# thu-wangz17/HermNet

Measured on AMD Instinct MI355X. Metric: atom-steps/sec (energy+forces) on 10k-atom 3-element cell; HBM GB/s vs roofline, higher is better.
Workload: dtype f32; 1 GPU; configs[1]: 10000-atom 3-element fcc alloy (Al/Ni/Cu), HVNet rc=5.0 hidden=128 num_rbf=128 layers=5, E=431340 directed edges, energy+forces per step; config=c2, atoms_total=10000, atoms_owned_rank0=10000, halo_atoms_rank0=0, edges_rank0=431340, tuned_gemm_table=False, gemm_tuning_in_warmup=False, parallelism=1 GPU

## Files before the change

### hermnet_amd/csrc/message_bwd_cl.hip

```cpp
#include <hip/hip_runtime.h>
#include <stdint.h>
#include <type_traits>
#include "../../include/hermnet_hip.h"
#include "hermnet_math.h"
#include "message_bwd_cl.h"

namespace {

typedef float hn_f2 __attribute__((ext_vector_type(2)));
typedef unsigned hn_u2 __attribute__((ext_vector_type(2)));
typedef __attribute__((address_space(4))) const float hn_cfloat;
typedef __attribute__((address_space(4))) const int hn_cint;

constexpr int kRec = HN_EDGE_TABLE_FLOATS;

#ifndef HN_NT_TABLE
#define HN_NT_TABLE 1
#endif
__device__ __forceinline__ float fwd_envelope_val(float u, int kind, int p) {
#pragma clang fp contract(off)
  if (kind != 0 || !(u < 1.0f)) return hn_envelope(u, kind, p).val;
  const float up = hn_powi(u, p - 1) * u;
  const float w = 1.0f - u;
  const float fp = (float)p;
// ... 332 lines not shown
    }
    for (int base = e_begin; base < e_end; base += 64) {
      const int cnt = min(64, e_end - base);
      const unsigned my_off = lane < cnt ? (unsigned)a.csc_tgt[base + lane] * (unsigned)(H * 4) : 0u;
      const int my_pos = lane < cnt ? a.csc_pos[base + lane] : 0;

      auto load_edge = [&](int k) {
        EdgeIn in;
        const unsigned so = (unsigned)__builtin_amdgcn_readlane((int)my_off, k);
        in.gx1 = buf_load(rs_gx1, c4, so);
        in.g0 = buf_load(rs_gvec1, c4, 3u * so);
        in.g1 = buf_load(rs_gvec1, c4, 3u * so + h4);
        in.g2 = buf_load(rs_gvec1, c4, 3u * so + 2 * h4);
        return in;
      };

      EdgeIn in0 = load_edge(0), in1 = in0;
      float px[2], py[2], pz[2];
      float ux[2], uy[2], uz[2];
      auto edge_body = [&](auto J, int k) {
        constexpr int j = decltype(J)::value;
        while (base + k >= row_end) {
          row_epilogue(row);
          ++row;
          row_end = row_end2;
          row_end2 = rowptr_c[min(row + 2, a.Nsrc)];
          row_request(row);
        }
        const int kn = j == 3 ? min(k + 1, 63) : k + 1;
        if (j & 1) in0 = load_edge(kn); else in1 = load_edge(kn);
        const EdgeIn& cur = (j & 1) ? in1 : in0;
        float (&tl)[5] = (j & 1) ? tl1 : tl0;
        hn_f2 Ss = {0.f, 0.f}, Sa = {0.f, 0.f}, Sb = {0.f, 0.f};
        auto taps4 = [&](int m0, const hn_f4 (&w)[4]) {
#pragma unroll
          for (int q = 0; q < 4; ++q) {
            const hn_f2 g = {rec[2 * (m0 + q)], rec[2 * (m0 + q) + 1]};
            Ss = __builtin_elementwise_fma(g, hn_f2{w[q].x, w[q].x}, Ss);
            if (HAS_VEC) Sa = __builtin_elementwise_fma(g, hn_f2{w[q].y, w[q].y}, Sa);
            Sb = __builtin_elementwise_fma(g, hn_f2{w[q].z, w[q].z}, Sb);
          }
        };
        lds_wait_all(wA, wB, wC);
#if HN_KO_BWD == 1
        Ss = hn_f2{rec[0] * wA[0].x, rec[1]}; Sa = hn_f2{rec[2] * wB[0].y, rec[3]}; Sb = hn_f2{rec[4] * wC[0].z, rec[5]};
#else
        taps4(0, wA);
        taps4(4, wB);
        taps4(8, wC);
#endif
        unsigned waddr_next;
        float own = 1.0f;
        if constexpr (WIN) {
          const int prow_next = __float_as_int(tl[0]);
          waddr_next = (unsigned)win_row(prow_next) * (HN_CB * 16) + tile_lane;
          own = own_cur ? 1.0f : 0.0f;
          own_mask = j == 0 ? own_cur : (own_mask | (own_cur << j));
          own_cur = win_owns(prow_next);
        } else {
          waddr_next = (unsigned)__float_as_int(tl[0]) * (HN_CB * 16) + tile_lane;
        }
        __builtin_amdgcn_sched_barrier(0);
        asm volatile("" : "+v"(Ss), "+v"(Sa), "+v"(Sb));
        rp += kRec;
        if (j & 1) load_record(tl0); else load_record(tl1);
        issue_weights(waddr_next);
        __builtin_amdgcn_sched_barrier(0);
        if (fresh) row_scale();
#if HN_KO_BWD == 2
        {
          gs += Ss.x + Ss.y + cur.gx1; ga += Sa.x + Sa.y + cur.g0; gb += Sb.x + Sb.y + cur.g1 + cur.g2;
          px[j & 1] = gs; py[j & 1] = ga; pz[j & 1] = gb;
          return;
        }
#endif
        const float rx = tl[1], ry = tl[2], rz = tl[3], invd = tl[4];
        const float gx1 = WIN ? cur.gx1 * own : cur.gx1, g0 = WIN ? cur.g0 * own : cur.g0;
        const float g1 = WIN ? cur.g1 * own : cur.g1, g2 = WIN ? cur.g2 * own : cur.g2;
        const float rs = Ss.x + bs;
        if (NEED_GXH) gs = fmaf(gx1, rs, gs);
        float pdv = gx1 * xs * Ss.y;
        if (HAS_VEC) {
          const float ra_ = Sa.x + ba;
          const float A = fmaf(g0, vj0, fmaf(g1, vj1, g2 * vj2));
          ga = fmaf(A, ra_, ga);
          const float w = xas * ra_;
          gv0 = fmaf(g0, w, gv0); gv1 = fmaf(g1, w, gv1); gv2 = fmaf(g2, w, gv2);
          pdv = fmaf(A * xa, Sa.y, pdv);
        }
        const float rb_ = Sb.x + bb;
        const float B = fmaf(rx, g0, fmaf(ry, g1, rz * g2));
        if (NEED_GXH) gb = fmaf(B, rb_, gb);
        pdv = fmaf(B * xb, Sb.y, pdv);
        const float qi = xb * rb_ * invd;
        const float tpar = fmaf(-B, qi, pdv);
        px[j & 1] = fmaf(tpar, rx, g0 * qi); py[j & 1] = fmaf(tpar, ry, g1 * qi); pz[j & 1] = fmaf(tpar, rz, g2 * qi);
      };
      auto fold = [&](int h) {
        ux[h] = pair_fold(px[0], px[1]); uy[h] = pair_fold(py[0], py[1]); uz[h] = pair_fold(pz[0], pz[1]);
      };
      auto group_store = [&](int k4) {
        const float sx = quad_total(ux[0], ux[1]), sy = quad_total(uy[0], uy[1]), sz = quad_total(uz[0], uz[1]);
        const int je = (row16 == 0) ? 0 : (row16 == 1 ? 2 : (row16 == 2 ? 1 : 3));
        const int p0 = __builtin_amdgcn_readlane(my_pos, k4), p1 = __builtin_amdgcn_readlane(my_pos, min(k4 + 1, cnt - 1));
        const int p2 = __builtin_amdgcn_readlane(my_pos, min(k4 + 2, cnt - 1)), p3 = __builtin_amdgcn_readlane(my_pos, min(k4 + 3, cnt - 1));
        const int pw = (row16 == 0) ? p0 : (row16 == 1 ? p2 : (row16 == 2 ? p1 : p3));
        if constexpr (WIN) {
          if ((lane & 15) == 0 && k4 + je < cnt && ((own_mask >> je) & 1u)) gedge[pw] = make_float4(sx, sy, sz, 0.f);
        } else {
#if HN_NT_MSG
          if ((lane & 15) == 0 && k4 + je < cnt)
            __builtin_nontemporal_store(hn_f4{sx, sy, sz, 0.f}, reinterpret_cast<hn_f4*>(&gedge[pw]));
#else
          if ((lane & 15) == 0 && k4 + je < cnt) gedge[pw] = make_float4(sx, sy, sz, 0.f);
// ... 202 lines not shown
```

### hermnet_amd/csrc/node_kernels.hip

```cpp
#include <hip/hip_runtime.h>
#include "../../include/hermnet_hip.h"

namespace {

constexpr float kInvSqrt2 = 0.70710678118654752f;
constexpr float kSiluScale = 1.0f / 0.6f;

__device__ __forceinline__ float4 ld4(const float* p) { return *reinterpret_cast<const float4*>(p); }
__device__ __forceinline__ void st4(float* p, float4 v) { *reinterpret_cast<float4*>(p) = v; }
__device__ __forceinline__ float sigmoidf_(float x) { return 1.0f / (1.0f + __expf(-x)); }


__device__ __forceinline__ float4 add4(float4 a, float4 b) { return make_float4(a.x + b.x, a.y + b.y, a.z + b.z, a.w + b.w); }

__device__ __forceinline__ float4 bias4(const float* bias, int rows_per_bias, long row, int cols, int col) {
  if (bias == nullptr) return make_float4(0.f, 0.f, 0.f, 0.f);
  const long grp = rows_per_bias > 0 ? row / rows_per_bias : 0;
  return ld4(bias + grp * cols + col);
}

__global__ __launch_bounds__(256) void ssilu_fwd_kernel(const float* __restrict__ h, const float* __restrict__ bias,
                                                        int rows_per_bias, float* __restrict__ a, long n4, int cols) {
  const long i = (long)blockIdx.x * blockDim.x + threadIdx.x;
  if (i >= n4) return;
// ... 457 lines not shown
                                                        const int* __restrict__ ranges, int num_ranges) {
  const int q4 = H;
  const long i = (long)blockIdx.x * blockDim.x + threadIdx.x;
  const long rows = MODE == 0 ? rows_out : (MODE == 1 ? (long)Te * P * B : (long)Te * B);
  if (i >= rows * q4) return;
  const long r = i / q4;
  if (MODE == 2 && num_ranges > 0) {
    bool in = false;
    for (int k = 0; k < num_ranges; ++k) in |= r >= ranges[2 * k] && r < ranges[2 * k + 1];
    if (!in) return;
  }
  const int c = (int)(i % q4) * 4;
  const float sc = c < H ? sx : sv;
  auto at = [&](const float* x, const float* v, long row) {
    return c < H ? ld4(x + row * H + c) : ld4(v + row * 3 * H + (c - H));
  };
  float* dst = c < H ? xout + r * H + c : vout + r * 3 * H + (c - H);
  if (MODE != 1) {
    float4 acc = make_float4(0.f, 0.f, 0.f, 0.f);
    if (r < (long)Te * B) {
      const long ce = r / B, ii = r % B;
      for (int k = 0; k < P; ++k) acc = add4(acc, at(xin, vin, (ce * P + k) * B + ii));
      acc = make_float4(acc.x * sc, acc.y * sc, acc.z * sc, acc.w * sc);
    }
    if (MODE == 2) acc = add4(acc, ld4(dst));
    st4(dst, acc);
  } else {
    const long ce = r / ((long)P * B), ii = r % B;
    const float4 g = at(xin, vin, ce * B + ii);
    st4(dst, make_float4(g.x * sc, g.y * sc, g.z * sc, g.w * sc));
  }
}

inline dim3 grid_for(long n, int block) { return dim3((unsigned)((n + block - 1) / block)); }
#define HN_LAUNCH_END return hipGetLastError() == hipSuccess ? HN_OK : HN_ERR_LAUNCH

}

extern "C" int hermnet_ssilu_fwd(const float* h, const float* bias, int rows_per_bias, float* a, long rows, int cols,
                                 void* stream) {
  if (rows < 0 || cols <= 0 || (cols & 3)) return HN_ERR_BAD_ARG;
  if (rows == 0) return HN_OK;
  if (!h || !a) return HN_ERR_BAD_ARG;
  const long n4 = rows * (cols / 4);
  hipLaunchKernelGGL(ssilu_fwd_kernel, grid_for(n4, 256), dim3(256), 0, (hipStream_t)stream, h, bias, rows_per_bias,
                     a, n4, cols);
  HN_LAUNCH_END;
}

extern "C" int hermnet_ssilu_bwd(const float* g, const float* h, const float* bias, int rows_per_bias, float* gh,
                                 int N, int T, int C, long g_stride_n, long g_stride_t, void* stream) {
  if (N < 0 || T <= 0 || C <= 0 || (C & 3) || (g_stride_n & 3) || (g_stride_t & 3)) return HN_ERR_BAD_ARG;
  if (N == 0) return HN_OK;
  if (!g || !h || !gh) return HN_ERR_BAD_ARG;
  hipLaunchKernelGGL(ssilu_bwd_kernel, grid_for((long)N * T * (C / 4), 256), dim3(256), 0, (hipStream_t)stream,
                     g, h, bias, rows_per_bias, gh, N, T, C, g_stride_n, g_stride_t);
  HN_LAUNCH_END;
}

extern "C" int hermnet_update_mid(const float* vp, const float* x1, float* vdot, float* xin, int rows, int hidden,
                                  void* stream) {
  if (rows < 0 || hidden <= 0 || (hidden & 3)) return HN_ERR_BAD_ARG;
  if (rows == 0) return HN_OK;
  if (!vp || !x1 || !vdot || !xin) return HN_ERR_BAD_ARG;
  hipLaunchKernelGGL(update_mid_kernel, grid_for((long)rows * (hidden / 4), 256), dim3(256), 0, (hipStream_t)stream,
                     vp, x1, vdot, xin, rows, hidden);
// ... 104 lines not shown
  };
  if (cols == 64) return go(energy_head_fused_kernel<true, 1>);
  if (cols == 128) return go(energy_head_fused_kernel<true, 2>);
  return go(energy_head_fused_kernel<true, 4>);
}

extern "C" int hermnet_energy_head_fused_bwd(const float* ge, const float* h, const float* w0, const float* w2,
                                             const float* row_mask, float* gx, int rows, int hidden, int cols,
                                             void* stream) {
  if (rows < 0 || (hidden != 64 && hidden != 128 && hidden != 256) || cols <= 0 || (cols & 3) ||
      (size_t)hidden * cols * 4 > 65536)
    return HN_ERR_BAD_ARG;
  if (rows == 0) return HN_OK;
  if (!ge || !h || !w0 || !w2 || !gx) return HN_ERR_BAD_ARG;
  const size_t lds = ((size_t)hidden * cols + 32 * (cols + 1)) * sizeof(float);
  const dim3 grid((unsigned)((rows + 31) / 32));
  hipStream_t s = (hipStream_t)stream;
  auto go = [&](auto kern) -> int {
    static bool done = false;
    if (!done) {
      if (hipFuncSetAttribute(reinterpret_cast<const void*>(kern), hipFuncAttributeMaxDynamicSharedMemorySize, 98304) != hipSuccess)
        return HN_ERR_LDS;
      done = true;
    }
    hipLaunchKernelGGL(kern, grid, dim3(256), lds, s, h, w0, (const float*)nullptr, w2, (const float*)nullptr, ge, row_mask,
                       gx, (float*)nullptr, rows, cols);
    HN_LAUNCH_END;
  };
  if (hidden == 64) return go(energy_head_fused_kernel<false, 1>);
  if (hidden == 128) return go(energy_head_fused_kernel<false, 2>);
  return go(energy_head_fused_kernel<false, 4>);
}

extern "C" int hermnet_pair_mean(int mode, const float* x_in, const float* vec_in, float* x_out, float* vec_out,
                                 int num_elem, int pairs, int block, int rows_out, int hidden, float scale_x,
                                 float scale_vec, const int* row_ranges, int num_ranges, void* stream) {
  if (num_elem < 0 || pairs <= 0 || block < 0 || hidden <= 0 || (hidden & 3) || rows_out < (long)num_elem * block ||
      mode < 0 || mode > 2 || num_ranges < 0 || (num_ranges > 0 && (!row_ranges || mode != 2)))
    return HN_ERR_BAD_ARG;
  const long rows = mode == 0 ? (long)rows_out : (mode == 1 ? (long)num_elem * pairs * block : (long)num_elem * block);
  if (rows == 0) return HN_OK;
  if (!x_in || !vec_in || !x_out || !vec_out) return HN_ERR_BAD_ARG;
  const dim3 grid = grid_for(rows * hidden, 256);
  hipStream_t s = (hipStream_t)stream;
  switch (mode) {
    case 0: hipLaunchKernelGGL(pair_mean_kernel<0>, grid, dim3(256), 0, s, x_in, vec_in, x_out, vec_out, num_elem, pairs, block, rows_out, hidden, scale_x, scale_vec, (const int*)nullptr, 0); break;
    case 1: hipLaunchKernelGGL(pair_mean_kernel<1>, grid, dim3(256), 0, s, x_in, vec_in, x_out, vec_out, num_elem, pairs, block, rows_out, hidden, scale_x, scale_vec, (const int*)nullptr, 0); break;
    default: hipLaunchKernelGGL(pair_mean_kernel<2>, grid, dim3(256), 0, s, x_in, vec_in, x_out, vec_out, num_elem, pairs, block, rows_out, hidden, scale_x, scale_vec, row_ranges, num_ranges); break;
  }
  HN_LAUNCH_END;
}

extern "C" int hermnet_halo_rows(int mode, float* x, float* vec, const long* idx, int n, int hidden, float* buf,
                                 void* stream) {
  if (n < 0 || hidden <= 0 || (hidden & 3) || mode < 0 || mode > 2) return HN_ERR_BAD_ARG;
  if (n == 0) return HN_OK;
  if (!x || !vec || !idx || !buf) return HN_ERR_BAD_ARG;
  const dim3 grid = grid_for((long)n * hidden, 256);
  hipStream_t s = (hipStream_t)stream;
  switch (mode) {
    case 0: hipLaunchKernelGGL(halo_rows_kernel<0>, grid, dim3(256), 0, s, x, vec, idx, n, hidden, buf); break;
    case 1: hipLaunchKernelGGL(halo_rows_kernel<1>, grid, dim3(256), 0, s, x, vec, idx, n, hidden, buf); break;
    case 2: hipLaunchKernelGGL(halo_rows_kernel<2>, grid, dim3(256), 0, s, x, vec, idx, n, hidden, buf); break;
    default: return HN_ERR_BAD_ARG;
  }
  HN_LAUNCH_END;
// ... 39 lines not shown
```

### hermnet_amd/hermnet.py

```python
from typing import Dict, List, Union

import torch
from torch import nn

from . import nodeops, switches
from .elements import atomic_numbers
from .ops import EdgeGeometry, TrueEdgeGradient, edge_radial_tables
from .relations import AtomSet, RelationalGraph
from .sharding import HaloExchange, HaloExchangeFeatures, HaloGradReturn, SumAcrossRanks
from .layer import (EdgeFanout, EdgeGradSink, EnergyHead, FusedRelationalLayer, GemmRelationalLayer, HeadWeights, LayerWeights,
                    Route, StepState)
from .rmnet import PaiNNModule, RadialBasis, ScaledSiLU, relational_layer
from .trainops import EdgeDiff, EdgeUnit, embedding_rows, tall_linear


class HeteroVertexConv(nn.Module):

    def __init__(self, mods: Dict[str, nn.Module]):
        super().__init__()
        self.mods = nn.ModuleDict(mods)
        self._weights = None

    def forward(self, data):
        step = data.get("_hn_step")
        if step is None:
            raise RuntimeError("HeteroVertexConv.forward needs a Data prepared by HVNet.forward")
        g, li = step.graph, step.layer
        halo, step.halo = step.halo, None
        ready = step.weights
        w = ready[li] if (ready is not None and ready[li].mods[0] is next(iter(self.mods.values()))) else None
        if w is None and step.edge_embed is None and switches.fused_layer:
            if self._weights is None:
                self._weights = LayerWeights(self.mods.values())
            w = self._weights.refresh()
        if halo is not None and _exchange_first(halo, w, g, data.x):
            data.x, data.vec = HaloExchangeFeatures.apply(data.x, data.vec, halo.plan)
            halo = None
        if step.edge_embed is not None:
            data.x, data.vec = relational_layer(self.mods.values(), data.x, data.vec, step.edge, g, None,
                                                edge_embed=step.edge_embed)
            return data
        if not switches.fused_layer:
            data.x, data.vec = relational_layer(self.mods.values(), data.x, data.vec, step.edge, g, step.rbf)
            return data
        edge = step.edge if step.edge_handles is None else step.edge_handles[li]
        node, step.chain_node = step.chain_node, None
        if not (w.chain and switches.node_chain):
            if halo is not None:
                raise RuntimeError("the in-layer halo exchange belongs to the chain path")
            data.x, data.vec = GemmRelationalLayer.apply(data.x, data.vec, edge, g, step.rbf, w, step)
            return data
        route = _chain_route(data, step, node, halo)
        data.x, data.vec = FusedRelationalLayer.apply(data.x, data.vec, edge, g, step.rbf, w, step, route)
        step.chain_node = None if g.num_src else data.x.grad_fn
        return data


def _exchange_first(halo, w, g, x):
    return not (w is not None and w.chain and switches.node_chain
                and halo.fwd_early is not None and g.N * 3 * x.size(1) * 4 < 2 ** 32
                and sum(halo.plan.recv_counts) + sum(halo.plan.send_counts) > 0
                and switches.halo_overlap() != "0")


def _chain_route(data, step, node, halo):
    g, li, ready = step.graph, step.layer, step.weights
    straight = (node is not None and data.vec is not None and data.x.grad_fn is node and data.vec.grad_fn is node
                and not g.num_src and not torch.is_anomaly_enabled()
                and not getattr(data.x, "_backward_hooks", None) and not getattr(data.vec, "_backward_hooks", None))
    if halo is not None:
        return Route("proj" if straight and switches.halo_overlap() not in ("0", "1") else "rows", halo)
    pre = step.pre_next.pop(li, None)
    if pre is not None and not (pre[0].data_ptr() == data.x.data_ptr() and pre[0].shape == data.x.shape):
        pre = None
    w_next = ready[li + 1] if (ready is not None and li + 1 < len(ready) and step.whole) else None
    last = step.last and not g.num_src and w_next is None
    return Route(defer=straight and step.whole, pre=None if pre is None else pre[1], w_next=w_next, last=last)


class GraphEnergies(torch.autograd.Function):

    @staticmethod
    def forward(ctx, e_rows, graph, batch):
        ctx.graph, ctx.batch, ctx.rows = graph, batch, e_rows.size(0)
        pa = e_rows.index_select(0, graph.row_of_node).index_select(0, graph.graph_perm)
        return torch.segment_reduce(pa, "sum", lengths=graph.graph_lengths, unsafe=True)

    @staticmethod
    def backward(ctx, ge):
        return _GraphSpread.apply(ge, ctx.graph, ctx.batch, ctx.rows), None, None


class _GraphSpread(torch.autograd.Function):
    @staticmethod
    def forward(ctx, ge, graph, batch, rows):
        ctx.graph, ctx.batch = graph, batch
        def make():
            idx = torch.zeros(rows, dtype=torch.long, device=ge.device).scatter_(0, graph.row_of_node, batch)
            real = torch.zeros(rows, dtype=ge.dtype, device=ge.device).scatter_(
                0, graph.row_of_node, torch.ones(graph.row_of_node.numel(), dtype=ge.dtype, device=ge.device))
            return idx, real
        idx, real = graph.derived("row_graph", make, key=rows)
        return ge.index_select(0, idx) * real

    @staticmethod
    def backward(ctx, c_rows):
        return GraphEnergies.apply(c_rows.contiguous(), ctx.graph, ctx.batch), None, None, None


MAX_PADDED_WIDTH = 1024
# ... 3 lines not shown

    def __init__(self, elems: Union[str, List[str]], rc: float = 5.,
                 intensive: bool = False, num_layers: int = 5,
                 hidden_channels: int = 512, num_rbf: int = 128,
                 rbf={"name": "gaussian"},
                 envelope={"name": "polynomial", "exponent": 5}):
        super().__init__()
        if isinstance(elems, str):
            elems = [elems]
        self.elems = list(elems)
        if (hidden_channels + 63) // 64 * 64 > MAX_PADDED_WIDTH:
            raise ValueError("hermnet_amd: hidden_channels = %d pads to %d channels; the LayerNorm kernels hold a row of at "
                             "most %d (csrc/node_kernels.hip: kLnMaxPerLane), so the widest model has hidden_channels = %d"
                             % (hidden_channels, (hidden_channels + 63) // 64 * 64, MAX_PADDED_WIDTH, MAX_PADDED_WIDTH))
        self.rc = rc
        self.num_layers = num_layers
        self.hidden_channels = hidden_channels
        self.intensive = intensive

        self.embed = nn.Embedding(len(atomic_numbers), hidden_channels)
        self.radial_basis = RadialBasis(num_radial=num_rbf, cutoff=rc, rbf=rbf, envelope=envelope)
        self.hermconvs = nn.ModuleList()
        for _ in range(num_layers):
            self.hermconvs.append(HeteroVertexConv(
                mods={ntype: PaiNNModule(hidden_channels=hidden_channels, num_rbf=num_rbf) for ntype in self.elems}))
        self.out_energy = nn.Sequential(
            nn.Linear(hidden_channels, hidden_channels // 2),
            ScaledSiLU(),
            nn.Linear(hidden_channels // 2, 1),
        )

    def invalidate_caches(self):
        self.__dict__["_cache_epoch"] = self.__dict__.get("_cache_epoch", 0) + 1
        for w in [getattr(conv, "_weights", None) for conv in self.hermconvs] + [self.__dict__.get("_head")]:
            if w is not None:
                w.key = None
        g = self.__dict__.get("_guard")
        if g is not None:
            g.armed_for, g._event = None, None
        return self

    def load_state_dict(self, *args, **kwargs):
        out = super().load_state_dict(*args, **kwargs)
        self.invalidate_caches()
        return out

    def _apply(self, fn, *args, **kwargs):
        out = super()._apply(fn, *args, **kwargs)
        if "hermconvs" in self._modules:
            self.invalidate_caches()
        return out

    def train(self, mode=True):
        if "hermconvs" in self._modules and mode != self.training:
            self.invalidate_caches()
        return super().train(mode)

    def _refresh_weights(self, dev):
        from .guard import ParamGuard
        guard_on = dev.type == "cuda" and switches.param_guard()
        for _ in range(2):
            ws = []
            for conv in self.hermconvs:
                if conv._weights is None:
                    conv._weights = LayerWeights(conv.mods.values())
                ws.append(conv._weights.refresh())
            hw = None
            if (self.hidden_channels // 2) % 4 == 0:
                if self.__dict__.get("_head") is None:
                    self.__dict__["_head"] = HeadWeights(self.out_energy)
                hw = self._head.refresh()
            if not guard_on or not ws:
                return ws, hw
            g = self.__dict__.get("_guard")
            if g is None:
                g = self.__dict__["_guard"] = ParamGuard(self)
            extra = tuple((p_.data_ptr(), p_._version) for p_ in (self.embed.weight, self.out_energy[0].weight,
                                                                 self.out_energy[0].bias, self.out_energy[2].weight,
                                                                 self.out_energy[2].bias))
            if not g.step(dev, tuple((id(w), w.builds) for w in ws + [hw] if w is not None) + extra, ws[0].b1cat):
                return ws, hw
            self.invalidate_caches()
        return ws, hw

    eval_param_grads = False

    @staticmethod
    def _require_device(pos):
        if not pos.is_cuda:
            raise RuntimeError("hermnet_amd.HVNet runs on MI355X only (data is on %s); there is no CPU fallback"
                               % pos.device)

    def _require_fp32(self, pos):
        wd = self.embed.weight.dtype
        if wd != torch.float32 or pos.dtype != torch.float32:
            raise TypeError("hermnet_amd.HVNet computes in float32: parameters are %s, data.pos is %s "
                            "(call model.float() / pos.float())" % (wd, pos.dtype))

    def _z_list(self):
        return [atomic_numbers[el] for el in self.elems]

    def atom_set(self, atomic_number, batch):
        return AtomSet.of(atomic_number, batch, self._z_list())

    def _build_graph(self, data, zl, shard, atoms):
        rel_active = None if shard is None else shard.rel_active(zl)
        return RelationalGraph.build(data.atomic_number, data.edge_index, zl,
                                     edge_shift=data.get("edge_shift") if data.get("cell") is not None else None,
                                     batch=data.batch, rel_active=rel_active, atoms=atoms)

    @staticmethod
    def _edge_geometry_autograd(pos, cell, graph):
        src = graph.src_id.long()
# ... 65 lines not shown
        if train and pos.is_cuda:
            x = embedding_rows(self.embed.weight, graph.z_rows.long())
        else:
            x = self.embed(graph.z_rows) if train else torch.nn.functional.embedding(graph.z_rows, self.embed.weight.detach())
        H = self.hidden_channels
        Hp = (H + 63) // 64 * 64 if (fused and switches.fused_layer) else H
        if Hp != H:
            x = torch.nn.functional.pad(x, (0, Hp - H))
        weights, head = self._refresh_weights(pos.device) if fused and switches.fused_layer else (None, None)
        if train:
            edge, edge_parts = self._edge_geometry_autograd(pos, data.get("cell"), graph)
        elif props is not None and (props.want_virials or props.want_graph_virial):
            edge = EdgeGeometry.apply(pos, data.get("cell"), graph, props)
        else:
            edge = EdgeGeometry.apply(pos, data.get("cell"), graph)
        if not fused and not train:
            edge = TrueEdgeGradient.apply(edge)
        graph.fwd_taps = None
        if fused and edge.requires_grad and edge.is_cuda:
            graph.edge_table, graph.fwd_taps = edge_radial_tables(graph, rbf, edge.detach())
        if fused:
            edge_embed = None
        elif train and pos.is_cuda and self.radial_basis.rbf_name == "gaussian" and H % 4 == 0 and graph.T > 0:
            parts, Ek = edge_parts, graph.rel_edge_total()
            edge_embed = self.radial_basis.bucketed(edge[:, 3] if parts is None else parts[1], Ek, graph.T,
                                                    graph.rel_edge_bounds_dev())
            if parts is not None:
                edge_embed.set_unit_vectors(edge, parts[0], Ek)
        else:
            edge_embed = self.radial_basis(edge[:, 3])
        data.x, data.vec = x, None
        data._hn_graph, data._hn_edge, data._hn_edge_embed = graph, edge, edge_embed
        step = StepState(graph, edge, rbf, edge_embed, train=train, fused=fused, whole=whole, weights=weights, head=head)
        if fused and edge.requires_grad and switches.fused_layer:
            all_known = graph.num_src == 0 and graph.N == graph.type_rowptr_host[-1]
            step.edge_sink = EdgeGradSink(len(self.hermconvs), Hp // 64, graph.E, pos.device, zero=not all_known)
            step.edge_handles = EdgeFanout.apply(edge, step.edge_sink)
        return step

    def _run_layers(self, data, step):
        graph, edge, L = step.graph, step.edge, len(self.hermconvs)
        for li, conv in enumerate(self.hermconvs):
            step.layer = li
            step.last = bool(li + 1 == L and step.fused and switches.fused_layer and switches.dead_ends
                             and type(conv) is HeteroVertexConv
                             and edge.requires_grad and not conv._forward_hooks
                             and not torch.nn.modules.module._global_forward_hooks)
            data = conv(data)
            if not step.whole and li + 1 < L:
                step.halo = data._hn_shard.halo_overlap(graph, nodeops.chain_tile_rows(data.x.size(1)) or 64)
        step.weights = step.edge_handles = step.halo = step.chain_node = None
        return data

    def _read_out(self, data, step):
        graph, shard, H = step.graph, data.get("_hn_shard"), self.hidden_channels
        x = data.x if data.x.size(1) == H else data.x[:, :H]
        head, step.head = step.head, None
        mask = graph.row_real if shard is None and graph.num_graphs == 1 else None
        if shard is not None and shard.num_graphs == 1 and head is not None:
            mask = shard.owned_rows(graph, x.size(0))
        e_rows = self._row_energies(x, step.train, head, mask)
        props = data.get("_hn_atom_props")
        if props is not None and props.want_energies:
            props.energies = self._atom_energies(e_rows, graph, data.batch)
        return self._graph_energies(e_rows, graph, data.batch, shard, mask is not None)

# ... 124 lines not shown
```

### hermnet_amd/layer.py

```python
import torch

from . import _lib, nodeops, switches
from .ops import _launch, _msg_bwd, _msg_bwd_gedge, _msg_fwd
from .sharding import _all_to_all_rows_start, comm_wait


class LayerWeights(object):

    STATE = ("mods", "key", "builds", "_params", "h_real", "chain")
    DENSE = ("w1cat", "b1cat", "w1cat_t", "w2", "w2t", "b2", "wt", "brbf", "wv", "wvt", "wx0", "wx0t", "bx0", "wx2", "wx2t",
             "bx2", "wv_s", "wvt_s", "wx0_s", "wx0t_s", "bx0_s", "wx2_s", "wx2t_s", "bx2_s")
    FRAG = ("w1f", "w1tf", "w2f", "w2tf", "wvf", "wvtf", "wx0f", "wx0tf", "wx2f", "wx2tf")
    FRAG16 = tuple(n + "16" for n in FRAG)
    __slots__ = STATE + DENSE + FRAG + FRAG16

    def __init__(self, mods):
        for n in self.__slots__:
            setattr(self, n, None)
        self.mods = list(mods)
        self.builds = 0
        self._params = [(sub, name) for m in self.mods for sub in m.modules() for name in sub._parameters]

    @property
    def __dict__(self):
# ... 73 lines not shown
    return tuple(key)


class HeadWeights(object):

    __slots__ = ("lin0", "lin2", "key", "builds", "w0", "b0", "w2v", "b2", "w0t", "w0f16", "w0tf16")

    def __init__(self, out_energy=None):
        for n in self.__slots__:
            setattr(self, n, None)
        if out_energy is not None:
            self.lin0, self.lin2 = out_energy[0], out_energy[2]
        self.builds = 0

    @torch.no_grad()
    def refresh(self):
        key = _version_key([(m, n) for m in (self.lin0, self.lin2) for n in ("weight", "bias")])
        if key != self.key:
            self.build(self.lin0.weight.detach(), self.lin0.bias.detach(), self.lin2.weight.detach(), self.lin2.bias.detach())
            self.key = key
            self.builds += 1
        return self

    def build(self, w0, b0, w2, b2):
        H, C = w0.size(1), w0.size(0)
        self.w0, self.b0, self.w2v, self.b2 = w0.contiguous(), b0, w2.reshape(-1).contiguous(), b2
        if nodeops.head16_supported(H, C):
            self.w0f16, self.w0tf16 = nodeops.weight_fragments16(self.w0), nodeops.weight_fragments16(self.w0.t().contiguous())
        elif nodeops.head_fused_supported(H, C):
            self.w0t = self.w0.t().contiguous()
        return self


def _bwd_sums_deferrable(graph, H):
    return (H == 128 and graph.edge_table is not None and not graph.num_src and graph.res_row is None
            and _lib.get_option("bwd_lanes16") == 0
            and graph.N * 3 * H * 4 < 2 ** 32 and switches.defer_sums())


def _virtual_residual(graph, gx1, gvec1, gx_in, gvec_in, H, ranges=None):
    if not graph.num_src:
        return
    P_, B_, Te = graph.triadic_pairs, graph.block, graph.T // graph.triadic_pairs
    if gx_in.is_cuda and gvec_in is not None:
        nodeops.pair_sum_accumulate(gx1, gvec1, gx_in, gvec_in, Te, P_, B_, 0.5 ** 0.5, 1.0, ranges=ranges)
        return
    sel = slice(0, Te * B_)
    if ranges is not None:
        sel = torch.zeros(Te * B_, dtype=torch.bool)
        for lo, hi in ranges[1]:
            sel[lo:min(hi, Te * B_)] = True
    gx_in[:Te * B_][sel] += (gx1.view(Te, P_, B_, H).sum(1).reshape(Te * B_, H) * (0.5 ** 0.5))[sel]
    if gvec_in is not None:
        gvec_in[:Te * B_][sel] += gvec1.view(Te, P_, B_, 3, H).sum(1).reshape(Te * B_, 3, H)[sel]


class EdgeGradSink(object):

    def __init__(self, layers, nblk, E, device, zero=True):
        self.shape = (layers, nblk, E, 4)
        self.device = device
        self.zero = zero
        self.buf = None

    def slice(self, li):
        if self.buf is None:
            alloc = torch.zeros if self.zero else torch.empty
            self.buf = alloc(self.shape, dtype=torch.float32, device=self.device)
            if not self.zero and switches.debug_poison():
                self.buf.fill_(float("nan"))
        return self.buf[li]


class EdgeFanout(torch.autograd.Function):

    @staticmethod
    def forward(ctx, edge, sink):
        ctx.sink = sink
        L, nblk = sink.shape[0], sink.shape[1]
        return tuple(edge.unsqueeze(0).expand(nblk, *edge.shape) for _ in range(L))

    @staticmethod
    def backward(ctx, *grads):
        sink = ctx.sink
        buf, ctx.sink.buf = sink.buf, None
        if buf is not None and all(g is not None and g.data_ptr() == buf[i].data_ptr() for i, g in enumerate(grads)):
            L, nblk, E, _ = sink.shape
            return buf.view(L * nblk, E, 4).sum(0), None
        live = [g.sum(0) for g in grads if g is not None]
        return (torch.stack(live, 0).sum(0) if live else None), None


class StepState(object):

    __slots__ = ("graph", "edge", "rbf", "edge_embed", "train", "fused", "whole", "weights", "head", "edge_sink",
                 "edge_handles", "layer", "last", "halo", "chain_node", "pending", "pre_next")

    def __init__(self, graph=None, edge=None, rbf=None, edge_embed=None, train=False, fused=False, whole=True, weights=None,
                 head=None):
        self.graph = graph
        self.edge = edge
        self.rbf = rbf
        self.edge_embed = edge_embed
        self.train = train
        self.fused = fused
        self.whole = whole
        self.weights = weights
        self.head = head
        self.edge_sink = None
        self.edge_handles = None
        self.layer = 0
        self.last = False
        self.halo = None
        self.chain_node = None
        self.pending = {}
        self.pre_next = {}


class Route(object):

    def __init__(self, exchange=None, halo=None, defer=False, pre=None, w_next=None, last=False):
        self.exchange, self.halo, self.defer, self.pre, self.w_next = exchange, halo, defer, pre, w_next
        self.boundary = int(switches.boundary_mode)
        self.first = bool(switches.dead_ends)
        self.last = bool(last and switches.dead_ends and exchange is None and w_next is None)


def _local_fwd(x, vec, edge, graph, rbf, w, route):
    pre = route.pre if route.pre is not None else nodeops.node_pre_fwd(x, w, graph.T, src_ranges=graph.src_ranges)
    x1, vec1 = _msg_fwd(graph, rbf, x.size(1), pre[1], vec, x, w, edge, xh_bias=False)
    return pre, x1, vec1


def _halo_rows_fwd(x, vec, edge, graph, rbf, w, route):
    halo, plan, H = route.halo, route.halo.plan, x.size(1)
    send = nodeops.halo_rows(0, x, vec, plan.send_idx)
    recv, work = _all_to_all_rows_start(send, plan.send_counts, plan.recv_counts, plan.group)
    if switches.debug_poison():
        nodeops.halo_rows(2, x, vec, plan.recv_idx, torch.full_like(recv, float("nan")))
    pre = nodeops.node_pre_fwd(x, w, graph.T, src_ranges=graph.src_ranges)
    out = _msg_fwd(graph, rbf, H, pre[1], vec, x, w, edge, xh_bias=False, ranges=halo.fwd_early, zero_unknown=True,
                   range_rows=halo.early_rows)
    comm_wait(work, "fwd", sum(plan.send_counts), sum(plan.recv_counts))
    if plan.recv_idx.numel() > 0:
        nodeops.halo_rows(2, x, vec, plan.recv_idx, recv)
        nodeops.node_pre_fwd(x, w, graph.T, src_ranges=graph.src_ranges, windows=halo.windows, mode=1, out=pre)
    if halo.late_rows > 0:
        _msg_fwd(graph, rbf, H, pre[1], vec, x, w, edge, xh_bias=False, ranges=halo.fwd_late, zero_unknown=False, out=out,
                 range_rows=halo.late_rows)
    return pre, out[0], out[1]


def _halo_proj_fwd(x, vec, edge, graph, rbf, w, route):
    halo, plan, H = route.halo, route.halo.plan, x.size(1)
    pre = nodeops.node_pre_fwd(x, w, graph.T, src_ranges=graph.src_ranges)
    xh = pre[1]
    send = nodeops.halo_proj_rows(0, xh, vec, plan.send_idx)
    recv, work = _all_to_all_rows_start(send, plan.send_counts, plan.recv_counts, plan.group)
    if switches.debug_poison():
        nodeops.halo_proj_rows(2, xh, vec, plan.recv_idx, torch.full_like(recv, float("nan")))
    out = _msg_fwd(graph, rbf, H, xh, vec, x, w, edge, xh_bias=False, ranges=halo.fwd_early, zero_unknown=True,
                   range_rows=halo.early_rows)
# ... 91 lines not shown
    return gx_total, gvec_in


def _halo_proj_bwd(ctx, x, mean, rstd, hb, xh, vec, edge, gx1, gvec1, gedge):
    graph, rbf, w, halo, plan, H = ctx.graph, ctx.rbf, ctx.w, ctx.route.halo, ctx.route.halo.plan, x.size(1)
    gxh = torch.empty_like(xh)
    gv_parts = torch.empty((graph.T,) + tuple(vec.shape), dtype=vec.dtype, device=vec.device)
    bufs = (gxh, gv_parts)
    if halo.bwd_first_rows[1]:
        _msg_bwd(graph, rbf, H, xh, vec, w, edge, gx1, gvec1, gedge, xh_bias=False, ranges=halo.bwd_first_rows, out=bufs,
                 finish=False)
    gsend = nodeops.halo_proj_rows(1, gxh, gv_parts, plan.recv_idx)
    back, work = _all_to_all_rows_start(gsend, plan.recv_counts, plan.send_counts, plan.group)
    if halo.bwd_rest_rows[1]:
        _msg_bwd(graph, rbf, H, xh, vec, w, edge, gx1, gvec1, gedge, xh_bias=False, ranges=halo.bwd_rest_rows, out=bufs,
                 finish=False)
    comm_wait(work, "bwd", sum(plan.recv_counts), sum(plan.send_counts))
    nodeops.halo_proj_accumulate(gxh, gv_parts, plan, back)
    gn_parts = nodeops.node_pre_bwd(gxh, hb, x, mean, rstd, w, src_ranges=graph.src_ranges, parts_only=True)
    return _hand_down(ctx.step, ctx.li, x, vec, gn_parts, gv_parts, mean, rstd, gx1, gvec1, w)


_ROUTES = {None: (_local_fwd, _local_bwd), "rows": (_halo_rows_fwd, _halo_rows_bwd), "proj": (_halo_proj_fwd, _halo_proj_bwd)}


class FusedRelationalLayer(torch.autograd.Function):

    @staticmethod
    def forward(ctx, x, vec, edge, graph, rbf, w, step, route):
        x = x.contiguous()
        vec = None if vec is None else vec.contiguous()
        ctx.exchange = "rows" if (route.exchange == "proj" and not _bwd_sums_deferrable(graph, x.size(1))
                                  and (ctx.needs_input_grad[0] or ctx.needs_input_grad[2])) else route.exchange
        (hb, xh, mean, rstd), x1, vec1 = _ROUTES[ctx.exchange][0](x, vec, edge, graph, rbf, w, route)
        ctx.short = route.last and x.is_cuda and ctx.exchange is None and nodeops.last_update_supported(graph, x.size(1), w)
        if ctx.short:
            x_out, vp, h2b, q23, nrm = nodeops.node_update_fwd_last(x1, vec1, w, graph)
            vec_out = None
        else:
            x_out, vec_out, vp, h2b, q23, nrm = _update_fwd(x1, vec1, graph, w, step, step.layer, route)
        ctx.save_for_backward(x, mean, rstd, hb, xh, vec, edge, vp, h2b, q23, nrm)
        ctx.graph, ctx.rbf, ctx.w, ctx.step, ctx.li, ctx.route = graph, rbf, w, step, step.layer, route
        return x_out, vec_out

    @staticmethod
    def backward(ctx, gxo, gvo):
        x, mean, rstd, hb, xh, vec, edge, vp, h2b, q23, nrm = ctx.saved_tensors
        pend = ctx.step.pending.pop(ctx.li, None)
        if ctx.short:
            if pend is not None:
                raise RuntimeError("hermnet_amd: gradients handed down to the last layer")
            gx1, gvec1 = nodeops.node_update_bwd_last(gxo.contiguous(), vp, h2b, q23, nrm, ctx.w, ctx.graph)
        else:
            gxo, gvo = gxo.contiguous(), gvo.contiguous()
            if pend is not None and (pend.gx.data_ptr() != gxo.data_ptr() or pend.gvec.data_ptr() != gvo.data_ptr()):
                raise RuntimeError("hermnet_amd: the gradients handed down as partial sums (layer %d) did not arrive in the "
                                   "buffers they were registered with; set the environment variable named in "
                                   "hermnet_amd/switches.py: defer_sums to 0" % (ctx.li + 1))
            gx1, gvec1 = nodeops.node_update_bwd(gxo, gvo, vp, h2b, q23, nrm, ctx.w, ctx.graph, pending=pend)
        gedge = _edge_grad_slot(edge, ctx.graph, ctx.step, ctx.li, x.size(1), gx1.device)
        gx, gvec = _ROUTES[ctx.exchange][1](ctx, x, mean, rstd, hb, xh, vec, edge, gx1, gvec1, gedge)
        return (gx, gvec, _edge_grad(edge, gedge)) + (None,) * 5


def _relation_gemms(graph, a, w_s, w_t, out, bias=None, acc=False):
    rp = graph.type_rowptr_host
# ... 107 lines not shown
```

### hermnet_amd/nodeops.py

```python

import ctypes

import torch

from . import _lib
from .ops import _call

P = _lib.ptr


def _new(like, *shape):
    return torch.empty(*shape, dtype=like.dtype, device=like.device)


def layernorm_fwd(x, eps=1e-5, h_real=0):
    rows, H = x.shape
    n, mean, rstd = _new(x, rows, H), _new(x, rows), _new(x, rows)
    _call("layernorm_fwd", "hermnet_layernorm_fwd", P(x), P(n), P(mean), P(rstd), rows, H, h_real, eps)
    return n, mean, rstd


def layernorm_bwd(g, x, mean, rstd, add=None, h_real=0):
    rows, H = x.shape
    gx = _new(x, rows, H)
# ... 179 lines not shown
def update_tile_rows(graph, H):
    return graph.derived("upd_tile", lambda: int(_lib.load().hermnet_node_update_tile_rows(
        _rowptr_host(graph), graph.N, graph.T, H)), key=H)


def update_stream(graph, H, w):
    if update_tile_rows(graph, H) == 16 and w.wvf16 is not None:
        return _stream16(w)
    return 0, (w.wvf, w.wx0f, w.wx2f), (w.wx2tf, w.wx0tf, w.wvtf)


def _stream16(w):
    return 16, (w.wvf16, w.wx0f16, w.wx2f16), (w.wx2tf16, w.wx0tf16, w.wvtf16)


def _rowptr_host(graph):
    return graph.derived("rowptr_c", lambda: (ctypes.c_int * len(graph.type_rowptr_host))(*graph.type_rowptr_host))


def _pre_outputs(x, T, zero_stats=False):
    Ns, H = x.shape
    alloc = torch.zeros if zero_stats else torch.empty
    hb, xh = _new(x, T, Ns, H), _new(x, T, Ns, 3 * H)
    return hb, xh, alloc(Ns, dtype=x.dtype, device=x.device), alloc(Ns, dtype=x.dtype, device=x.device)


def node_pre_fwd(x, w, T, src_ranges=None, windows=None, mode=0, out=None):
    Ns, H = x.shape
    hb, xh, mean, rstd = out if out is not None else _pre_outputs(x, T, zero_stats=src_ranges is not None)
    nwin = 0 if windows is None else int(windows.size(0))
    _call("node_pre_fwd", "hermnet_node_pre_fwd", P(x), P(w.w1f), P(w.b1cat), P(w.w2f), P(w.b2), P(hb), P(xh), P(mean),
          P(rstd), P(src_ranges), Ns, T, H, w.h_real, 1e-5, P(windows), nwin, mode if windows is not None else 0)
    return hb, xh, mean, rstd


def node_pre_bwd(gxh, hb, x, mean, rstd, w, add=None, src_ranges=None, windows=None, mode=0, out=None, parts_only=False):
    T, Ns, H = hb.shape
    if parts_only:
        x = mean = rstd = add = windows = out = None
    parts, gx = (out[1], out[0]) if out is not None else (_new(hb, T, Ns, H), None if parts_only else torch.empty_like(x))
    nwin = 0 if windows is None else int(windows.size(0))
    _call("node_pre_bwd", "hermnet_node_pre_bwd", P(gxh), P(hb), P(w.w2tf), P(w.w1tf), P(parts), P(x), P(mean), P(rstd),
          P(add), P(gx), P(src_ranges), Ns, T, H, w.h_real, P(windows), nwin, mode if windows is not None else 0)
    if parts_only:
        return parts
    return gx if out is None and windows is None else (gx, parts)


def _update_outputs(x1, vec_out=True):
    N, H = x1.shape
    return (_new(x1, N, 3, 2 * H), _new(x1, N, H), _new(x1, N, 2 * H), _new(x1, N, H), _new(x1, N, H),
            _new(x1, N, 3, H) if vec_out else None)


def _update_fwd(form, x1, vec1, w, graph, w_next=None):
    N, H = x1.shape
    tile, (wvf, wx0f, wx2f), _ = update_stream(graph, H, w) if form == "general" else _stream16(w)
    vp, h2b, q23, nrm, xo, vo = _update_outputs(x1, vec_out=form != "last")
    args = (P(x1), P(vec1), P(wvf), P(wx0f), P(w.bx0_s), P(wx2f), P(w.bx2_s), P(graph.row_active), P(graph.type_rowptr),
            _rowptr_host(graph), P(vp), P(h2b), P(q23), P(nrm), P(xo))
    pre = None
    if form == "general":
        _call("node_update_fwd", "hermnet_node_update_fwd", *args, P(vo), N, graph.T, H, tile)
    elif form == "last":
        _call("node_update_fwd", "hermnet_node_update_fwd_last", *args, N, graph.T, H)
    else:
# ... 79 lines not shown
```

### hermnet_amd/switches.py

```python
import os

fused_layer = True
node_chain = True
boundary_mode = 0
native_relations = True
dead_ends = True
train_row_sums = True


def _env(name, default):
    return os.environ.get("HERMNET_" + name, default)


def debug_poison():
    return _env("DEBUG_POISON", "0") != "0"


def halo_overlap():
    return _env("HALO_OVERLAP", "2")


def defer_sums():
    return _env("DEFER_SUMS", "1") != "0"


def param_guard():
    return _env("PARAM_GUARD", "1") != "0"
```

### include/hermnet_hip.h

```cpp
#ifndef HERMNET_HIP_H
#define HERMNET_HIP_H

#include <stddef.h>

#ifdef __cplusplus
extern "C" {
#endif

#define HN_OK 0
#define HN_ERR_BAD_ARG 1
#define HN_ERR_LDS 2
#define HN_ERR_LAUNCH 3

#define HN_ENV_POLYNOMIAL 0
#define HN_ENV_EXPONENTIAL 1

#define HN_ABI_VERSION 13
int hermnet_abi_version(void);
const char* hermnet_build_info(void);

#define HN_OPT_FWD_ROWS 4
#define HN_OPT_BWD_ROWS 5
#define HN_OPT_BWD_CL_ROWS 6
#define HN_OPT_BWD_LANES16 7
// ... 156 lines not shown
                           const float* qbias, int rows_per_bias, const float* vdot,
                           const float* vp, const float* row_mask, float* gq, float* gvdot, float* gvp,
                           float* gx1, float* gvec1, int num_nodes, int num_known, int hidden, void* stream);
int hermnet_update_mid_bwd(const float* gvdot, const float* gxin, const float* vp, const float* xin,
                           float* gvp, float* gx1, int rows, int hidden, void* stream);

int hermnet_energy_head_fwd(const float* h, const float* w, const float* b, const float* row_mask, float* e,
                            int rows, int cols, void* stream);
int hermnet_energy_head_bwd(const float* ge, const float* h, const float* w, const float* row_mask, float* gh,
                            int rows, int cols, void* stream);

int hermnet_energy_head_fused_fwd(const float* x, const float* w0t, const float* b0, const float* w2, const float* b2,
                                  const float* row_mask, float* h, float* e, int rows, int hidden, int cols,
                                  void* stream);
int hermnet_energy_head_fused_bwd(const float* ge, const float* h, const float* w0, const float* w2,
                                  const float* row_mask, float* gx, int rows, int hidden, int cols, void* stream);

int hermnet_energy_head16_supported(int hidden, int cols);
int hermnet_energy_head16_fwd(const float* x, const float* w0_frag16, const float* b0, const float* w2, const float* b2,
                              const float* row_mask, float* h, float* e, int rows, int hidden, int cols, void* stream);
int hermnet_energy_head16_bwd(const float* ge, const float* h, const float* w0t_frag16, const float* w2,
                              const float* row_mask, float* gx, int rows, int hidden, int cols, void* stream);

int hermnet_node_chain_supported(int hidden);
int hermnet_node_chain_tile_rows(int hidden, int update);
int hermnet_node_pre_fwd(const float* x, const float* w1_frag, const float* b1, const float* w2_frag, const float* b2,
                         float* hb, float* xh, float* mean, float* rstd, const int* src_ranges, int num_src,
                         int num_rel, int hidden, int hidden_real, float eps, const int* row_windows, int num_windows,
                         int window_mode, void* stream);
int hermnet_node_pre_bwd(const float* gxh, const float* hb, const float* w2t_frag, const float* w1t_frag,
                         float* gn_parts, const float* x, const float* mean, const float* rstd, const float* add,
                         float* gx, const int* src_ranges, int num_src, int num_rel, int hidden, int hidden_real,
                         const int* row_windows, int num_windows, int window_mode, void* stream);
typedef struct hn_pending_grads {
  const float* gn_parts;
  const float* gvec_parts;
  const float* x;
  const float* mean;
  const float* rstd;
  const float* gx1;
  const float* gvec1;
  int num_parts;
  int hidden_real;
  const float* gxh;
  const float* hb;
  const float* w2t_frag16;
  const float* w1t_frag16;
} hn_pending_grads;
int hermnet_node_update_tile_rows(const int* type_rowptr_host, int num_nodes, int num_rel, int hidden);
int hermnet_node_update_fwd(const float* x1, const float* vec1, const float* wv_frag, const float* wx0_frag,
                            const float* bx0, const float* wx2_frag, const float* bx2, const float* row_active,
                            const int* type_rowptr, const int* type_rowptr_host, float* vp, float* h2b, float* q23,
                            float* nrm, float* x_out, float* vec_out, int num_nodes, int num_rel, int hidden,
                            int tile_rows, void* stream);
int hermnet_node_update_bwd(const float* gx_out, const float* gvec_out, const float* vp, const float* h2b,
                            const float* q23, const float* nrm, const float* wx2t_frag, const float* wx0t_frag,
                            const float* wvt_frag,
                            const float* row_active, const int* type_rowptr, const int* type_rowptr_host, float* gx1,
                            float* gvec1, int num_nodes, int num_rel, int hidden, int tile_rows,
                            const hn_pending_grads* pending, void* stream);

int hermnet_node_update_fwd_last(const float* x1, const float* vec1, const float* wv_frag16, const float* wx0_frag16,
                                 const float* bx0, const float* wx2_frag16, const float* bx2, const float* row_active,
                                 const int* type_rowptr, const int* type_rowptr_host, float* vp, float* h2b, float* q23,
                                 float* nrm, float* x_out, int num_nodes, int num_rel, int hidden, void* stream);
int hermnet_node_update_bwd_last(const float* gx_out, const float* vp, const float* h2b, const float* q23,
// ... 166 lines not shown
```

Measured before the change: 3.824 million atom-steps/s.

## Precompute per-species layer-0 node pre-projection table and expand by species index

In inference mode, the first layer's node pre-projection depends only on the atom species embedding, so it is computed once per species into a cached table. At run time the table is gathered per atom by a new expand kernel instead of running node_pre_fwd over all atoms. Separately, the message backward kernel drops the unused Ss.x accumulation when NEED_GXH is false, which cuts FMAs and register pressure. The table is rebuilt when weights change and only applies when input gradients are not needed, but forces need gradients with respect to positions, not x, so it may still run.

```diff
diff --git a/hermnet_amd/csrc/message_bwd_cl.hip b/hermnet_amd/csrc/message_bwd_cl.hip
--- a/hermnet_amd/csrc/message_bwd_cl.hip
+++ b/hermnet_amd/csrc/message_bwd_cl.hip
@@ -388,11 +388,13 @@
         const EdgeIn& cur = (j & 1) ? in1 : in0;
         float (&tl)[5] = (j & 1) ? tl1 : tl0;
         hn_f2 Ss = {0.f, 0.f}, Sa = {0.f, 0.f}, Sb = {0.f, 0.f};
+        float sy = 0.f;
         auto taps4 = [&](int m0, const hn_f4 (&w)[4]) {
 #pragma unroll
           for (int q = 0; q < 4; ++q) {
             const hn_f2 g = {rec[2 * (m0 + q)], rec[2 * (m0 + q) + 1]};
-            Ss = __builtin_elementwise_fma(g, hn_f2{w[q].x, w[q].x}, Ss);
+            if constexpr (NEED_GXH) Ss = __builtin_elementwise_fma(g, hn_f2{w[q].x, w[q].x}, Ss);
+            else sy = __builtin_fmaf(g.y, w[q].x, sy);
             if (HAS_VEC) Sa = __builtin_elementwise_fma(g, hn_f2{w[q].y, w[q].y}, Sa);
             Sb = __builtin_elementwise_fma(g, hn_f2{w[q].z, w[q].z}, Sb);
           }
@@ -400,6 +402,7 @@
         lds_wait_all(wA, wB, wC);
 #if HN_KO_BWD == 1
         Ss = hn_f2{rec[0] * wA[0].x, rec[1]}; Sa = hn_f2{rec[2] * wB[0].y, rec[3]}; Sb = hn_f2{rec[4] * wC[0].z, rec[5]};
+        sy = Ss.y;
 #else
         taps4(0, wA);
         taps4(4, wB);
@@ -417,7 +420,8 @@
           waddr_next = (unsigned)__float_as_int(tl[0]) * (HN_CB * 16) + tile_lane;
         }
         __builtin_amdgcn_sched_barrier(0);
-        asm volatile("" : "+v"(Ss), "+v"(Sa), "+v"(Sb));
+        if constexpr (NEED_GXH) asm volatile("" : "+v"(Ss), "+v"(Sa), "+v"(Sb));
+        else asm volatile("" : "+v"(sy), "+v"(Sb));
         rp += kRec;
         if (j & 1) load_record(tl0); else load_record(tl1);
         issue_weights(waddr_next);
@@ -425,7 +429,7 @@
         if (fresh) row_scale();
 #if HN_KO_BWD == 2
         {
-          gs += Ss.x + Ss.y + cur.gx1; ga += Sa.x + Sa.y + cur.g0; gb += Sb.x + Sb.y + cur.g1 + cur.g2;
+          gs += Ss.x + Ss.y + sy + cur.gx1; ga += Sa.x + Sa.y + cur.g0; gb += Sb.x + Sb.y + cur.g1 + cur.g2;
           px[j & 1] = gs; py[j & 1] = ga; pz[j & 1] = gb;
           return;
         }
@@ -433,9 +437,8 @@
         const float rx = tl[1], ry = tl[2], rz = tl[3], invd = tl[4];
         const float gx1 = WIN ? cur.gx1 * own : cur.gx1, g0 = WIN ? cur.g0 * own : cur.g0;
         const float g1 = WIN ? cur.g1 * own : cur.g1, g2 = WIN ? cur.g2 * own : cur.g2;
-        const float rs = Ss.x + bs;
-        if (NEED_GXH) gs = fmaf(gx1, rs, gs);
-        float pdv = gx1 * xs * Ss.y;
+        if constexpr (NEED_GXH) gs = fmaf(gx1, Ss.x + bs, gs);
+        float pdv = gx1 * xs * (NEED_GXH ? Ss.y : sy);
         if (HAS_VEC) {
           const float ra_ = Sa.x + ba;
           const float A = fmaf(g0, vj0, fmaf(g1, vj1, g2 * vj2));
diff --git a/hermnet_amd/csrc/node_kernels.hip b/hermnet_amd/csrc/node_kernels.hip
--- a/hermnet_amd/csrc/node_kernels.hip
+++ b/hermnet_amd/csrc/node_kernels.hip
@@ -513,6 +513,22 @@
   }
 }
 
+template <typename I>
+__global__ __launch_bounds__(256) void species_expand_kernel(const float* __restrict__ table, const long* __restrict__ z_rows,
+                                                             float* __restrict__ xh, long rows, int V, int q4) {
+  const I n = (I)rows * (I)q4;
+  const I j = (I)blockIdx.x * 256u + threadIdx.x;
+  if (j >= n) return;
+  const I r = j / (I)q4;
+  const int c = (int)(j - r * (I)q4);
+  const long t = blockIdx.y;
+  long z = z_rows[r];
+  z = z < 0 ? 0 : (z >= V ? V - 1 : z);
+  const float4 v = reinterpret_cast<const float4*>(table)[(t * V + z) * q4 + c];
+  float4* dst = reinterpret_cast<float4*>(xh) + ((size_t)t * (size_t)rows * (size_t)q4 + (size_t)j);
+  *dst = v;
+}
+
 inline dim3 grid_for(long n, int block) { return dim3((unsigned)((n + block - 1) / block)); }
 #define HN_LAUNCH_END return hipGetLastError() == hipSuccess ? HN_OK : HN_ERR_LAUNCH
 
@@ -683,6 +699,24 @@
   return go(energy_head_fused_kernel<false, 4>);
 }
 
+extern "C" int hermnet_species_expand(const float* table, const long* z_rows, float* xh, int num_rows, int num_rel,
+                                      int num_species, int width, void* stream) {
+  if (num_rows < 0 || num_rel <= 0 || num_species <= 0 || width <= 0 || (width & 3)) return HN_ERR_BAD_ARG;
+  if (num_rows == 0) return HN_OK;
+  if (!table || !z_rows || !xh) return HN_ERR_BAD_ARG;
+  const long per_rel = (long)num_rows * (width / 4);
+  const long blocks = (per_rel + 255) / 256;
+  if (blocks > 0x7fffffffL || num_rel > 65535) return HN_ERR_BAD_ARG;
+  const dim3 grid((unsigned)blocks, (unsigned)num_rel);
+  if (per_rel < (1L << 32) - 256)
+    hipLaunchKernelGGL(species_expand_kernel<unsigned>, grid, dim3(256), 0, (hipStream_t)stream, table, z_rows, xh,
+                       (long)num_rows, num_species, width / 4);
+  else
+    hipLaunchKernelGGL(species_expand_kernel<unsigned long>, grid, dim3(256), 0, (hipStream_t)stream, table, z_rows, xh,
+                       (long)num_rows, num_species, width / 4);
+  HN_LAUNCH_END;
+}
+
 extern "C" int hermnet_pair_mean(int mode, const float* x_in, const float* vec_in, float* x_out, float* vec_out,
                                  int num_elem, int pairs, int block, int rows_out, int hidden, float scale_x,
                                  float scale_vec, const int* row_ranges, int num_ranges, void* stream) {
diff --git a/hermnet_amd/hermnet.py b/hermnet_amd/hermnet.py
--- a/hermnet_amd/hermnet.py
+++ b/hermnet_amd/hermnet.py
@@ -9,7 +9,7 @@
 from .relations import AtomSet, RelationalGraph
 from .sharding import HaloExchange, HaloExchangeFeatures, HaloGradReturn, SumAcrossRanks
 from .layer import (EdgeFanout, EdgeGradSink, EnergyHead, FusedRelationalLayer, GemmRelationalLayer, HeadWeights, LayerWeights,
-                    Route, StepState)
+                    Route, SpeciesTable, StepState)
 from .rmnet import PaiNNModule, RadialBasis, ScaledSiLU, relational_layer
 from .trainops import EdgeDiff, EdgeUnit, embedding_rows, tall_linear
 
@@ -50,7 +50,9 @@
                 raise RuntimeError("the in-layer halo exchange belongs to the chain path")
             data.x, data.vec = GemmRelationalLayer.apply(data.x, data.vec, edge, g, step.rbf, w, step)
             return data
-        route = _chain_route(data, step, node, halo)
+        plain = (type(self) is HeteroVertexConv and not self._forward_hooks and not self._forward_pre_hooks
+                 and not torch.nn.modules.module._global_forward_hooks and not torch.nn.modules.module._global_forward_pre_hooks)
+        route = _chain_route(data, step, node, halo, plain)
         data.x, data.vec = FusedRelationalLayer.apply(data.x, data.vec, edge, g, step.rbf, w, step, route)
         step.chain_node = None if g.num_src else data.x.grad_fn
         return data
@@ -63,7 +65,7 @@
                 and switches.halo_overlap() != "0")
 
 
-def _chain_route(data, step, node, halo):
+def _chain_route(data, step, node, halo, plain=False):
     g, li, ready = step.graph, step.layer, step.weights
     straight = (node is not None and data.vec is not None and data.x.grad_fn is node and data.vec.grad_fn is node
                 and not g.num_src and not torch.is_anomaly_enabled()
@@ -75,7 +77,11 @@
         pre = None
     w_next = ready[li + 1] if (ready is not None and li + 1 < len(ready) and step.whole) else None
     last = step.last and not g.num_src and w_next is None
-    return Route(defer=straight and step.whole, pre=None if pre is None else pre[1], w_next=w_next, last=last)
+    species = None
+    if (li == 0 and plain and step.species is not None and data.x is step.species[1] and data.vec is None and step.whole
+            and not step.train and not g.num_src and switches.species_table):
+        species = (step.species[0], g.z_rows)
+    return Route(defer=straight and step.whole, pre=None if pre is None else pre[1], w_next=w_next, last=last, species=species)
 
 
 class GraphEnergies(torch.autograd.Function):
@@ -145,7 +151,8 @@
 
     def invalidate_caches(self):
         self.__dict__["_cache_epoch"] = self.__dict__.get("_cache_epoch", 0) + 1
-        for w in [getattr(conv, "_weights", None) for conv in self.hermconvs] + [self.__dict__.get("_head")]:
+        for w in [getattr(conv, "_weights", None) for conv in self.hermconvs] + [self.__dict__.get("_head"),
+                                                                                 self.__dict__.get("_species")]:
             if w is not None:
                 w.key = None
         g = self.__dict__.get("_guard")
@@ -183,6 +190,11 @@
                 if self.__dict__.get("_head") is None:
                     self.__dict__["_head"] = HeadWeights(self.out_energy)
                 hw = self._head.refresh()
+            sp = None
+            if ws and dev.type == "cuda" and not self.training and ws[0].chain and switches.node_chain:
+                if self.__dict__.get("_species") is None:
+                    self.__dict__["_species"] = SpeciesTable(self.embed)
+                sp = self._species.refresh(ws[0])
             if not guard_on or not ws:
                 return ws, hw
             g = self.__dict__.get("_guard")
@@ -191,7 +203,7 @@
             extra = tuple((p_.data_ptr(), p_._version) for p_ in (self.embed.weight, self.out_energy[0].weight,
                                                                  self.out_energy[0].bias, self.out_energy[2].weight,
                                                                  self.out_energy[2].bias))
-            if not g.step(dev, tuple((id(w), w.builds) for w in ws + [hw] if w is not None) + extra, ws[0].b1cat):
+            if not g.step(dev, tuple((id(w), w.builds) for w in ws + [hw, sp] if w is not None) + extra, ws[0].brbf):
                 return ws, hw
             self.invalidate_caches()
         return ws, hw
@@ -323,6 +335,9 @@
         data.x, data.vec = x, None
         data._hn_graph, data._hn_edge, data._hn_edge_embed = graph, edge, edge_embed
         step = StepState(graph, edge, rbf, edge_embed, train=train, fused=fused, whole=whole, weights=weights, head=head)
+        sp = self.__dict__.get("_species")
+        if weights is not None and sp is not None and sp.table is not None and sp.key is not None and not train:
+            step.species = (sp.table, x)
         if fused and edge.requires_grad and switches.fused_layer:
             all_known = graph.num_src == 0 and graph.N == graph.type_rowptr_host[-1]
             step.edge_sink = EdgeGradSink(len(self.hermconvs), Hp // 64, graph.E, pos.device, zero=not all_known)
diff --git a/hermnet_amd/layer.py b/hermnet_amd/layer.py
--- a/hermnet_amd/layer.py
+++ b/hermnet_amd/layer.py
@@ -129,6 +129,31 @@
         return self
 
 
+class SpeciesTable(object):
+
+    __slots__ = ("embed", "key", "builds", "table")
+
+    def __init__(self, embed):
+        self.embed, self.key, self.builds, self.table = embed, None, 0, None
+
+    @torch.no_grad()
+    def refresh(self, w0):
+        key = _version_key([(self.embed, "weight")]) + ((id(w0), w0.builds),)
+        if key == self.key:
+            return self
+        emb = self.embed.weight.detach()
+        self.table = None
+        if not (w0.chain and emb.is_cuda and emb.dtype == torch.float32) or torch.cuda.is_current_stream_capturing():
+            return self
+        Hp = w0.b2.size(-1) // 3
+        if Hp != emb.size(1):
+            emb = torch.nn.functional.pad(emb, (0, Hp - emb.size(1)))
+        self.table = nodeops.species_table(emb.contiguous(), w0, len(w0.mods))
+        self.key = key
+        self.builds += 1
+        return self
+
+
 def _bwd_sums_deferrable(graph, H):
     return (H == 128 and graph.edge_table is not None and not graph.num_src and graph.res_row is None
             and _lib.get_option("bwd_lanes16") == 0
@@ -191,7 +216,7 @@
 class StepState(object):
 
     __slots__ = ("graph", "edge", "rbf", "edge_embed", "train", "fused", "whole", "weights", "head", "edge_sink",
-                 "edge_handles", "layer", "last", "halo", "chain_node", "pending", "pre_next")
+                 "edge_handles", "layer", "last", "halo", "chain_node", "pending", "pre_next", "species")
 
     def __init__(self, graph=None, edge=None, rbf=None, edge_embed=None, train=False, fused=False, whole=True, weights=None,
                  head=None):
@@ -212,19 +237,26 @@
         self.chain_node = None
         self.pending = {}
         self.pre_next = {}
+        self.species = None
 
 
 class Route(object):
 
-    def __init__(self, exchange=None, halo=None, defer=False, pre=None, w_next=None, last=False):
+    def __init__(self, exchange=None, halo=None, defer=False, pre=None, w_next=None, last=False, species=None):
         self.exchange, self.halo, self.defer, self.pre, self.w_next = exchange, halo, defer, pre, w_next
+        self.species = species if exchange is None and pre is None else None
         self.boundary = int(switches.boundary_mode)
         self.first = bool(switches.dead_ends)
         self.last = bool(last and switches.dead_ends and exchange is None and w_next is None)
 
 
 def _local_fwd(x, vec, edge, graph, rbf, w, route):
-    pre = route.pre if route.pre is not None else nodeops.node_pre_fwd(x, w, graph.T, src_ranges=graph.src_ranges)
+    if route.pre is not None:
+        pre = route.pre
+    elif route.species is not None:
+        pre = (None, nodeops.species_expand(route.species[0], route.species[1], x.size(0)), None, None)
+    else:
+        pre = nodeops.node_pre_fwd(x, w, graph.T, src_ranges=graph.src_ranges)
     x1, vec1 = _msg_fwd(graph, rbf, x.size(1), pre[1], vec, x, w, edge, xh_bias=False)
     return pre, x1, vec1
 
@@ -382,6 +414,8 @@
         vec = None if vec is None else vec.contiguous()
         ctx.exchange = "rows" if (route.exchange == "proj" and not _bwd_sums_deferrable(graph, x.size(1))
                                   and (ctx.needs_input_grad[0] or ctx.needs_input_grad[2])) else route.exchange
+        if route.species is not None and (ctx.needs_input_grad[0] or vec is not None or not x.is_cuda):
+            route.species = None
         (hb, xh, mean, rstd), x1, vec1 = _ROUTES[ctx.exchange][0](x, vec, edge, graph, rbf, w, route)
         ctx.short = route.last and x.is_cuda and ctx.exchange is None and nodeops.last_update_supported(graph, x.size(1), w)
         if ctx.short:
diff --git a/hermnet_amd/nodeops.py b/hermnet_amd/nodeops.py
--- a/hermnet_amd/nodeops.py
+++ b/hermnet_amd/nodeops.py
@@ -235,6 +235,21 @@
     _call("node_pre_fwd", "hermnet_node_pre_fwd", P(x), P(w.w1f), P(w.b1cat), P(w.w2f), P(w.b2), P(hb), P(xh), P(mean),
           P(rstd), P(src_ranges), Ns, T, H, w.h_real, 1e-5, P(windows), nwin, mode if windows is not None else 0)
     return hb, xh, mean, rstd
+
+
+def species_table(emb, w, T):
+    from .ops import _stream
+    hb, xh, mean, rstd = _pre_outputs(emb, T)
+    _lib.call("hermnet_node_pre_fwd", P(emb), P(w.w1f), P(w.b1cat), P(w.w2f), P(w.b2), P(hb), P(xh), P(mean), P(rstd), None,
+              emb.size(0), T, emb.size(1), w.h_real, 1e-5, None, 0, 0, _stream())
+    return xh
+
+
+def species_expand(table, z_rows, Ns):
+    T, V, W = table.shape
+    xh = _new(table, T, Ns, W)
+    _call("node_pre_fwd", "hermnet_species_expand", P(table), P(z_rows), P(xh), Ns, T, V, W)
+    return xh
 
 
 def node_pre_bwd(gxh, hb, x, mean, rstd, w, add=None, src_ranges=None, windows=None, mode=0, out=None, parts_only=False):
diff --git a/hermnet_amd/switches.py b/hermnet_amd/switches.py
--- a/hermnet_amd/switches.py
+++ b/hermnet_amd/switches.py
@@ -5,6 +5,7 @@
 boundary_mode = 0
 native_relations = True
 dead_ends = True
+species_table = True
 train_row_sums = True
 
 
diff --git a/include/hermnet_hip.h b/include/hermnet_hip.h
--- a/include/hermnet_hip.h
+++ b/include/hermnet_hip.h
@@ -212,6 +212,8 @@
                          float* gn_parts, const float* x, const float* mean, const float* rstd, const float* add,
                          float* gx, const int* src_ranges, int num_src, int num_rel, int hidden, int hidden_real,
                          const int* row_windows, int num_windows, int window_mode, void* stream);
+int hermnet_species_expand(const float* table, const long* z_rows, float* xh, int num_rows, int num_rel, int num_species,
+                           int width, void* stream);
 typedef struct hn_pending_grads {
   const float* gn_parts;
   const float* gvec_parts;
```

New measurement: 3.869 million atom-steps/s (median of 6 runs). 1.2% higher.
